# christhetree/mod_extraction

Hardware: NVIDIA B200
Metric: audio_seconds_rendered_per_second (higher is better)
Workload: dtype f32

## Files before the change

### mod_extraction_b200/csrc/phaser.cu

```cuda
#include "common.cuh"

namespace modfx {
namespace {

constexpr int kStagesAP = 6;
constexpr int kUpd = 4;
constexpr int kChunk = 128;
constexpr int kCtl = kChunk / kUpd;
constexpr int kState = 7;
constexpr int kMapFloats = 8 * kState;
constexpr int kSFloats = 8;

struct PhaserArgs {
    const float* x;
    float* y;
    int N;
    float sr;
    const float *rate, *depth, *centre, *feedback, *mix;
    int block;
    const int32_t* index;
    int n_items;
    int n_ctl;
    int n_chunks;
};

__device__ __forceinline__ int example_of(const PhaserArgs& a, int item) { return a.index ? a.index[item] : item; }

__device__ __forceinline__ float cascade_step(float in, float (&w)[kStagesAP], float c) {
    float v = in;
#pragma unroll
    for (int k = 0; k < kStagesAP; ++k) {
        const float y = fmaf(c, v, w[k]);
        w[k] = fmaf(-c, y, v);
        v = y;
    }
    return v;
}

__device__ __forceinline__ void cascade_retune(float (&w)[kStagesAP], float c_old, float c_new) {
    const float r = __fdividef(1.0f - c_new, 1.0f - c_old);
#pragma unroll
    for (int k = 0; k < kStagesAP; ++k) w[k] *= r;
}

__device__ __forceinline__ float2 cascade_step2(float2 in, float2 (&w)[kStagesAP], float c) {
    const float2 c2 = make_float2(c, c), nc2 = make_float2(-c, -c);
    float2 v = in;
#pragma unroll
    for (int k = 0; k < kStagesAP; ++k) {
        const float2 y = __ffma2_rn(c2, v, w[k]);
        w[k] = __ffma2_rn(nc2, y, v);
        v = y;
    }
    return v;
}

__device__ __forceinline__ void cascade_retune2(float2 (&w)[kStagesAP], float c_old, float c_new) {
    const float r = __fdividef(1.0f - c_new, 1.0f - c_old);
    const float2 r2 = make_float2(r, r);
#pragma unroll
    for (int k = 0; k < kStagesAP; ++k) w[k] = __fmul2_rn(w[k], r2);
}

constexpr int kSegChunks = 32;
constexpr int kSeg = kSegChunks * kChunk;
constexpr int kSub = 64;
constexpr int kSubs = kSeg / kSub;
constexpr int kSubCtl = kSub / kUpd;
constexpr int kSegCtl = kSeg / kUpd;
constexpr int kFusedThreads = 256;
constexpr int kRec = 8;

struct FusedArgs {
    PhaserArgs a;
    const int32_t* start;
    int n_out;
    float* dry_out;
    int x_compact;
    const int64_t* x_offset;
    int n_seg;
    int* ticket;
    int* flags;
    float* rec;
    float2* ph;
    float* phc;
};

__device__ __forceinline__ float phase_advance(float p, float inc, float two_pi) {
    const float next = p + inc;
    const float wrapped = next - two_pi;
    return (next >= two_pi) ? wrapped : next;
}

__global__ void __launch_bounds__(128) phaser_phase_kernel(const FusedArgs f, int n_blocks) {
    const PhaserArgs& a = f.a;
    const int pair = blockIdx.x * blockDim.x + threadIdx.x;
    if (pair >= a.n_items * n_blocks) return;
    const int item = pair / n_blocks, blk = pair - item * n_blocks;
    const int b = example_of(a, item);
    const int need = f.start ? min(a.N, f.start[b] + f.n_out) : a.N;
    if ((int64_t)blk * a.block >= need) return;
    const float two_pi = MODFX_TWO_PI_F;
    const float sr_down = (float)((double)a.sr / (double)kUpd);
    const float inc = a.rate[b] * (two_pi / sr_down);
    float p = 0.0f;
    for (int i = 0; i < blk; ++i) {
        const int n_down = ((i + 1) * a.block + kUpd - 1) / kUpd - (i * a.block + kUpd - 1) / kUpd;
        float next = __fadd_rn(p, __fmul_rn(inc, (float)n_down));
        while (next >= two_pi) next -= two_pi;
        p = next;
    }
    const int s0 = blk * a.block, s1 = min(s0 + a.block, a.N);
    if (f.phc) {
        float* out = f.phc + (int64_t)item * a.n_ctl;
        for (int j = (s0 + kUpd - 1) / kUpd; j < (s1 + kUpd - 1) / kUpd; ++j) {
            out[j] = p;
            float next = p + inc;
            while (next >= two_pi) next -= two_pi;
            p = next;
        }
        return;
    }
    const int c0 = s0 / kChunk, c1 = (s1 + kChunk - 1) / kChunk;
    float2* out = f.ph + (int64_t)item * a.n_chunks;
    float prev = 0.0f;
    const bool small = inc < two_pi;
    for (int c = c0; c < c1; ++c) {
        out[c].x = p;
        if (c > c0 || blk == 0) out[c].y = prev;
        if (small) {
#pragma unroll 8
            for (int j = 0; j < kCtl; ++j) {
                prev = p;
                p = phase_advance(p, inc, two_pi);
            }
        } else {
            for (int j = 0; j < kCtl; ++j) {
                prev = p;
                float next = p + inc;
                while (next >= two_pi) next -= two_pi;
                p = next;
            }
        }
    }
    if (s1 - s0 == a.block && c1 < a.n_chunks) out[c1].y = prev;
}

__device__ __forceinline__ float phaser_coef(float phase, float vol, float ctr, float log_span, float log_min, float w0) {
    float lfo = sinf(phase - MODFX_PI_F) * vol + ctr;
    lfo = fminf(fmaxf(lfo, 0.0f), 1.0f);
    const float fc = exp10f(lfo * log_span + log_min);
    const float g = tanf(w0 * fc);
    return 2.0f * (g / (1.0f + g)) - 1.0f;
}

__global__ void __launch_bounds__(kFusedThreads) phaser_fused_kernel(const FusedArgs f) {
    extern __shared__ __align__(16) float sm[];
    float(*xs)[kSub + 1] = reinterpret_cast<float(*)[kSub + 1]>(sm);
    float(*cs)[kSubCtl + 1] = reinterpret_cast<float(*)[kSubCtl + 1]>(sm + kSubs * (kSub + 1));
    float(*Ms)[kMapFloats + 1] = reinterpret_cast<float(*)[kMapFloats + 1]>(sm + kSubs * (kSub + 1) + kSubs * (kSubCtl + 1));
    float(*Ss)[kSFloats] = reinterpret_cast<float(*)[kSFloats]>(sm + kSubs * (kSub + 1) + kSubs * (kSubCtl + 1) + kSubs * (kMapFloats + 1));
    float* phs = reinterpret_cast<float*>(Ms);
    __shared__ int tile_s;
    __shared__ float entry[kRec];
    const PhaserArgs& a = f.a;
    const int tid = threadIdx.x, lane = tid & 31, warp = tid >> 5;
    if (tid == 0) tile_s = atomicAdd(f.ticket, 1);
    __syncthreads();
    const int tile = tile_s;
    const int seg = tile / a.n_items, item = tile - seg * a.n_items;
    const int b = example_of(a, item);
    const int start = f.start ? f.start[b] : 0;
    const int need = min(a.N, start + f.n_out);
    const int n_base = seg * kSeg;
    if (n_base >= need) return;
    const float* xr = f.x_offset ? a.x + f.x_offset[item] : a.x + (int64_t)(f.x_compact ? item : b) * a.N;
    const int row_len = f.x_offset ? need : a.N;

    const bool vec = ((reinterpret_cast<uintptr_t>(xr) & 15) == 0) && (n_base + kSeg <= row_len);
    if (vec) {
#pragma unroll
        for (int k = 0; k < kSeg / 4 / kFusedThreads; ++k) {
            const int i4 = tid + k * kFusedThreads;
            const float4 v = __ldg(reinterpret_cast<const float4*>(xr + n_base) + i4);
            float* d = &xs[i4 >> 4][(i4 & 15) << 2];
            d[0] = v.x; d[1] = v.y; d[2] = v.z; d[3] = v.w;
        }
    } else {
        for (int i = tid; i < kSeg; i += kFusedThreads) {
            const int n = n_base + i;
            xs[i / kSub][i % kSub] = (n < row_len) ? __ldg(xr + n) : 0.0f;
        }
    }
    const float two_pi = MODFX_TWO_PI_F;
    if (f.phc) {
        const float* pr = f.phc + (int64_t)item * a.n_ctl;
        for (int i = tid; i <= kSegCtl; i += kFusedThreads) {
            const int j = seg * kSegCtl - 1 + i;
            phs[i] = (j >= 0 && j < a.n_ctl) ? pr[j] : 0.0f;
        }
    } else if (tid < kSegChunks) {
        const int chunk = seg * kSegChunks + tid;
        const float sr_down = (float)((double)a.sr / (double)kUpd);
        const float inc = a.rate[b] * (two_pi / sr_down);
        float2 pp = (chunk < a.n_chunks) ? f.ph[(int64_t)item * a.n_chunks + chunk] : make_float2(0.0f, 0.0f);
        if (tid == 0) phs[0] = pp.y;
        float p = pp.x;
        if (inc < two_pi) {
#pragma unroll 8
            for (int q = 0; q < kCtl; ++q) {
                phs[1 + tid * kCtl + q] = p;
                p = phase_advance(p, inc, two_pi);
            }
        } else {
            for (int q = 0; q < kCtl; ++q) {
                phs[1 + tid * kCtl + q] = p;
                float next = p + inc;
                while (next >= two_pi) next -= two_pi;
                p = next;
            }
        }
    }
    __syncthreads();
    {
        const float f_lo = 20.0f;
        const double f_hi_d = (0.49 * (double)a.sr < 20000.0) ? 0.49 * (double)a.sr : 20000.0;
        const float log_min = log10f(f_lo), log_span = log10f((float)f_hi_d) - log_min;
        const float w0 = MODFX_PI_F / a.sr;
        const float vol = a.depth[b] * 0.5f;
        const float ctr = (log10f(a.centre[b]) - log_min) / log_span;
        float cv[(kSegCtl + 1 + kFusedThreads - 1) / kFusedThreads];
#pragma unroll
        for (int k = 0; k < (kSegCtl + 1 + kFusedThreads - 1) / kFusedThreads; ++k) {
            const int j = tid + k * kFusedThreads;
            cv[k] = (j <= kSegCtl) ? phaser_coef(phs[j], vol, ctr, log_span, log_min, w0) : 0.0f;
        }
        __syncthreads();
#pragma unroll
        for (int k = 0; k < (kSegCtl + 1 + kFusedThreads - 1) / kFusedThreads; ++k) {
            const int j = tid + k * kFusedThreads;
            if (j <= kSegCtl) {
                if (j >= 1) cs[(j - 1) / kSubCtl][1 + (j - 1) % kSubCtl] = cv[k];
                if (j % kSubCtl == 0 && j < kSegCtl) cs[j / kSubCtl][0] = cv[k];
            }
        }
    }
    __syncthreads();
    const float fbk = a.feedback[b];
    {
        const int pair = warp >> 1, sc = ((warp & 1) << 5) | lane;
        float2 s[kStagesAP];
#pragma unroll
        for (int k = 0; k < kStagesAP; ++k) s[k] = make_float2((2 * pair == k) ? 1.0f : 0.0f, (2 * pair + 1 == k) ? 1.0f : 0.0f);
        float2 out_prev = make_float2(0.0f, 0.0f);
        const float2 nfb = make_float2(-fbk, -fbk);
        float c_cur = cs[sc][0];
        int g0 = 0;
        if (pair == 3) {
            const float c0 = cs[sc][1];
            out_prev = cascade_step2(make_float2(-1.0f, xs[sc][0]), s, c0);
#pragma unroll
            for (int q = 1; q < kUpd; ++q)
                out_prev = cascade_step2(__ffma2_rn(nfb, out_prev, make_float2(0.0f, xs[sc][q])), s, c0);
            c_cur = c0;
            g0 = 1;
        }
#pragma unroll 2
        for (int g = g0; g < kSubCtl; ++g) {
            const float c = cs[sc][1 + g];
            cascade_retune2(s, c_cur, c);
            c_cur = c;
#pragma unroll
            for (int q = 0; q < kUpd; ++q) {
                const float2 u = (pair == 3) ? __ffma2_rn(nfb, out_prev, make_float2(0.0f, xs[sc][g * kUpd + q]))
                                             : __fmul2_rn(nfb, out_prev);
                out_prev = cascade_step2(u, s, c);
            }
        }
        float* m = &Ms[sc][2 * pair * kState];
#pragma unroll
        for (int k = 0; k < kStagesAP; ++k) {
            m[k] = s[k].x;
            m[kState + k] = s[k].y;
        }
        m[6] = out_prev.x * fbk;
        m[kState + 6] = out_prev.y * fbk;
    }
    __syncthreads();
    float(*GM)[kMapFloats + 1] = reinterpret_cast<float(*)[kMapFloats + 1]>(Ss + kSubs);
    float(*GS)[kSFloats] = reinterpret_cast<float(*)[kSFloats]>(reinterpret_cast<float*>(GM) + 8 * (kMapFloats + 1));
    {
        const int r = lane & 7, i0 = lane >> 3, i1 = i0 + 4;
        float* g = GM[warp];
        {
            const float* m = Ms[warp * 8];
            g[r * kState + i0] = m[r * kState + i0];
            if (i1 < kState) g[r * kState + i1] = m[r * kState + i1];
        }
        __syncwarp();
#pragma unroll 1
        for (int k = 1; k < 8; ++k) {
            const float* m = Ms[warp * 8 + k];
            float a0 = (r == 7) ? m[7 * kState + i0] : 0.0f;
            float a1 = (r == 7 && i1 < kState) ? m[7 * kState + i1] : 0.0f;
#pragma unroll
            for (int j = 0; j < kState; ++j) {
                const float cj = g[r * kState + j];
                a0 = fmaf(m[j * kState + i0], cj, a0);
                if (i1 < kState) a1 = fmaf(m[j * kState + i1], cj, a1);
            }
            __syncwarp();
            g[r * kState + i0] = a0;
            if (i1 < kState) g[r * kState + i1] = a1;
            __syncwarp();
        }
    }
    __syncthreads();
    if (warp == 0) {
        float* rec = f.rec + ((int64_t)item * f.n_seg + seg) * kRec;
        if (seg > 0) {
            const int* flag = f.flags + (int64_t)item * f.n_seg + seg - 1;
            if (lane == 0) {
                while (atomicAdd(const_cast<int*>(flag), 0) == 0) __nanosleep(64);
                __threadfence();
            }
            __syncwarp();
            if (lane < kRec) entry[lane] = __ldcg(rec - kRec + lane);
        } else if (lane < kRec) {
            entry[lane] = 0.0f;
        }
        __syncwarp();
        const int i = lane & 7, ii = (i < kState) ? i : 0;
        float sv = (i < kState) ? entry[i] : 0.0f;
        if (lane < 8) {
#pragma unroll 1
            for (int gq = 0; gq < 8; ++gq) {
                GS[gq][i] = sv;
                const float* m = GM[gq];
                float acc = m[7 * kState + ii];
#pragma unroll
                for (int r = 0; r < kState; ++r) acc = fmaf(m[r * kState + ii], __shfl_sync(0xffu, sv, r, 8), acc);
                sv = (i < kState) ? acc : 0.0f;
            }
            if (i < kState) rec[i] = sv;
            else rec[7] = cs[kSubs - 1][kSubCtl];
            __threadfence();
        }
        __syncwarp();
        if (lane == 0) atomicExch(f.flags + (int64_t)item * f.n_seg + seg, 1);
    }
    if (f.dry_out) {
        float* dr = f.dry_out + (int64_t)b * f.n_out;
        for (int i = tid; i < kSeg; i += kFusedThreads) {
            const int idx = n_base + i - start;
            if (idx >= 0 && idx < f.n_out && n_base + i < row_len) dr[idx] = xs[i / kSub][i % kSub];
        }
    }
    __syncthreads();
    if (lane < 8) {
        const int i = lane, ii = (i < kState) ? i : 0;
        float sv = (i < kState) ? GS[warp][i] : 0.0f;
#pragma unroll 1
        for (int k = 0; k < 8; ++k) {
            const int sc = warp * 8 + k;
            Ss[sc][i] = sv;
            const float* m = Ms[sc];
            float acc = m[7 * kState + ii];
#pragma unroll
            for (int r = 0; r < kState; ++r) acc = fmaf(m[r * kState + ii], __shfl_sync(0xffu, sv, r, 8), acc);
            sv = (i < kState) ? acc : 0.0f;
        }
    }
    __syncthreads();
    if (tid < kSubs) {
        const int sc = tid;
        float s[kStagesAP];
#pragma unroll
        for (int k = 0; k < kStagesAP; ++k) s[k] = Ss[sc][k];
        float last = Ss[sc][6];
        const float wet = a.mix[b], dry = 1.0f - a.mix[b];
        float c_cur = cs[sc][0];
#pragma unroll 2
        for (int g = 0; g < kSubCtl; ++g) {
            const float c = cs[sc][1 + g];
            cascade_retune(s, c_cur, c);
            c_cur = c;
#pragma unroll
            for (int q = 0; q < kUpd; ++q) {
                const float in = xs[sc][g * kUpd + q];
                const float out = cascade_step(in - last, s, c);
                last = out * fbk;
                xs[sc][g * kUpd + q] = fminf(fmaxf(fmaf(wet, out, dry * in), -1.0f), 1.0f);
            }
        }
    }
    __syncthreads();
    float* yr = a.y + (int64_t)b * f.n_out;
    if (vec && start == 0 && n_base + kSeg <= f.n_out && ((reinterpret_cast<uintptr_t>(yr) & 15) == 0)) {
#pragma unroll
        for (int k = 0; k < kSeg / 4 / kFusedThreads; ++k) {
            const int i4 = tid + k * kFusedThreads;
            const float* d = &xs[i4 >> 4][(i4 & 15) << 2];
            reinterpret_cast<float4*>(yr + n_base)[i4] = make_float4(d[0], d[1], d[2], d[3]);
        }
    } else {
        for (int i = tid; i < kSeg; i += kFusedThreads) {
            const int n = n_base + i;
            const int idx = n - start;
            if (idx >= 0 && idx < f.n_out && n < a.N) yr[idx] = xs[i / kSub][i % kSub];
        }
    }
}

int64_t align_up(int64_t v, int64_t a) { return (v + a - 1) / a * a; }

}
}

using namespace modfx;

extern "C" int64_t modfx_phaser_workspace_bytes(int32_t B, int64_t N) {
    if (B <= 0 || N <= 0) return 0;
    const int64_t n_ctl = (N + kUpd - 1) / kUpd, n_chunks = (N + kChunk - 1) / kChunk;
    const int64_t n_seg = (N + kSeg - 1) / kSeg;
    const int64_t phase_bytes = (n_ctl * 4 > n_chunks * 8) ? n_ctl * 4 : n_chunks * 8;
    return 256 + align_up((int64_t)B * n_seg * 4, 256) + align_up((int64_t)B * n_seg * kRec * 4, 256) +
           align_up((int64_t)B * phase_bytes, 256) + 256;
}

namespace {

int phaser_launch(const float* x, int x_compact, const int64_t* x_offset, float* y, float* dry_out, int32_t B, int64_t N, int64_t n_out, const int32_t* start,
                  float sr, const float* rate_hz, const float* depth, const float* centre_hz, const float* feedback,
                  const float* mix, int32_t block, const int32_t* example_index, int32_t n_items, void* workspace,
                  void* stream) {
    MODFX_REQUIRE(x && y && rate_hz && depth && centre_hz && feedback && mix, "NULL pointer");
    MODFX_REQUIRE(B >= 0 && N >= 1 && N < (1ll << 30), "bad shape B=%d N=%lld", B, (long long)N);
    MODFX_REQUIRE(n_out >= 1 && n_out <= N, "bad output window n_out=%lld (row length %lld)", (long long)n_out, (long long)N);
    MODFX_REQUIRE(sr > 0.0f, "sample rate must be positive");
    if (block <= 0) block = 8192;
    PhaserArgs a{};
    a.x = x; a.y = y; a.N = (int)N; a.sr = sr;
    a.rate = rate_hz; a.depth = depth; a.centre = centre_hz; a.feedback = feedback; a.mix = mix;
    a.block = block;
    a.index = example_index;
    a.n_items = example_index ? n_items : B;
    if (a.n_items == 0) return MODFX_OK;
    MODFX_REQUIRE(a.n_items > 0 && workspace, "workspace is NULL or n_items=%d", a.n_items);
    a.n_ctl = (int)((N + kUpd - 1) / kUpd);
    a.n_chunks = (int)((N + kChunk - 1) / kChunk);
    cudaStream_t s = as_stream(stream);
    char* w = static_cast<char*>(workspace);
    const int n_blocks = (int)((N + block - 1) / block);

    FusedArgs f{};
    f.a = a;
    f.start = start; f.n_out = (int)n_out; f.dry_out = dry_out; f.x_compact = x_compact; f.x_offset = x_offset;
    f.n_seg = (int)((N + kSeg - 1) / kSeg);
    f.ticket = reinterpret_cast<int*>(w);                                     w += 256;
    f.flags = reinterpret_cast<int*>(w);
    const int64_t flag_bytes = align_up((int64_t)a.n_items * f.n_seg * 4, 256);  w += flag_bytes;
    f.rec = reinterpret_cast<float*>(w);                                      w += align_up((int64_t)a.n_items * f.n_seg * kRec * 4, 256);
    if (block % kChunk == 0) f.ph = reinterpret_cast<float2*>(w);
    else f.phc = reinterpret_cast<float*>(w);
    MODFX_CUDA_OK(cudaMemsetAsync(workspace, 0, (size_t)(256 + flag_bytes), s));
    const int pairs = a.n_items * n_blocks;
    phaser_phase_kernel<<<(pairs + 127) / 128, 128, 0, s>>>(f, n_blocks);
    const size_t smem = sizeof(float) * (size_t)(kSubs * (kSub + 1) + kSubs * (kSubCtl + 1) + kSubs * (kMapFloats + 1) + kSubs * kSFloats +
                                                 8 * (kMapFloats + 1) + 8 * kSFloats);
    const int64_t tiles = (int64_t)a.n_items * f.n_seg;
    MODFX_REQUIRE(tiles < (1ll << 31), "too many segments in one call");
    phaser_fused_kernel<<<(unsigned)tiles, kFusedThreads, smem, s>>>(f);
    MODFX_CUDA_OK(cudaGetLastError());
    return MODFX_OK;
}

}

extern "C" int modfx_phaser_f32(const float* x, float* y, int32_t B, int64_t N, float sr, const float* rate_hz,
                                const float* depth, const float* centre_hz, const float* feedback,
                                const float* mix, int32_t block, const int32_t* example_index, int32_t n_items,
                                void* workspace, void* stream) {
    return phaser_launch(x, 0, nullptr, y, nullptr, B, N, N, nullptr, sr, rate_hz, depth, centre_hz, feedback, mix, block, example_index,
                         n_items, workspace, stream);
}

extern "C" int modfx_phaser_crop_f32(const float* x, int32_t x_compact, float* y, float* dry_out, int32_t B, int64_t N,
                                     int64_t n_out, const int32_t* start, float sr, const float* rate_hz, const float* depth,
                                     const float* centre_hz, const float* feedback, const float* mix, int32_t block,
                                     const int32_t* example_index, int32_t n_items, void* workspace, void* stream) {
    MODFX_REQUIRE(start, "start is NULL");
    MODFX_REQUIRE(!x_compact || example_index, "x_compact needs an example_index list");
    return phaser_launch(x, x_compact ? 1 : 0, nullptr, y, dry_out, B, N, n_out, start, sr, rate_hz, depth, centre_hz, feedback, mix, block, example_index,
                         n_items, workspace, stream);
}

extern "C" int modfx_phaser_crop_packed_f32(const float* x, const int64_t* x_offset, float* y, float* dry_out, int32_t B,
                                            int64_t N_max, int64_t n_out, const int32_t* start, float sr, const float* rate_hz,
                                            const float* depth, const float* centre_hz, const float* feedback, const float* mix,
                                            int32_t block, const int32_t* example_index, int32_t n_items, void* workspace,
                                            void* stream) {
    MODFX_REQUIRE(start && x_offset, "start or x_offset is NULL");
    MODFX_REQUIRE(example_index, "a packed x needs an example_index list (row i belongs to example example_index[i])");
    return phaser_launch(x, 1, x_offset, y, dry_out, B, N_max, n_out, start, sr, rate_hz, depth, centre_hz, feedback, mix, block,
                         example_index, n_items, workspace, stream);
}
```

Measured before the change: 1.214 million.

## Split final phaser replay into two pieces per sub-chunk and precompute retune ratios

Retune ratios are precomputed once into shared memory, so the per-step division in the transfer-map pass goes away. The map pass also records boundary states at the sub-chunk midpoint. These are combined with the entry state so that two warps replay the final wet pass in parallel per sub-chunk, each covering half the length. Segments that lie entirely before the start offset now return early, and the launch bound requests 5 blocks per SM. The cost is more register pressure from the boundary state arrays, extra shared-memory partial sums, and one more barrier.

New measurement: 1.245 million (median of 6 runs). 1.03x the previous value.

```diff
diff --git a/mod_extraction_b200/csrc/phaser.cu b/mod_extraction_b200/csrc/phaser.cu
--- a/mod_extraction_b200/csrc/phaser.cu
+++ b/mod_extraction_b200/csrc/phaser.cu
@@ -55,8 +55,7 @@
     return v;
 }
 
-__device__ __forceinline__ void cascade_retune2(float2 (&w)[kStagesAP], float c_old, float c_new) {
-    const float r = __fdividef(1.0f - c_new, 1.0f - c_old);
+__device__ __forceinline__ void cascade_rescale2(float2 (&w)[kStagesAP], float r) {
     const float2 r2 = make_float2(r, r);
 #pragma unroll
     for (int k = 0; k < kStagesAP; ++k) w[k] = __fmul2_rn(w[k], r2);
@@ -68,6 +67,9 @@
 constexpr int kSubs = kSeg / kSub;
 constexpr int kSubCtl = kSub / kUpd;
 constexpr int kSegCtl = kSeg / kUpd;
+constexpr int kPieces = 2;
+constexpr int kPieceLen = kSub / kPieces;
+constexpr int kPieceCtl = kSubCtl / kPieces;
 constexpr int kFusedThreads = 256;
 constexpr int kRec = 8;
 
@@ -154,7 +156,32 @@
     return 2.0f * (g / (1.0f + g)) - 1.0f;
 }
 
-__global__ void __launch_bounds__(kFusedThreads) phaser_fused_kernel(const FusedArgs f) {
+template <bool kAudio>
+__device__ __forceinline__ void map_runs(float2 (&s)[kStagesAP], float2& out_prev, int g0, const float* xrow,
+                                         const float* crow, const float* rcol, float fbk, float2 (&bd)[kPieces - 1][kState]) {
+    const float2 nfb = make_float2(-fbk, -fbk);
+#pragma unroll
+    for (int pc = 0; pc < kPieces; ++pc) {
+#pragma unroll 1
+        for (int g = (pc == 0) ? g0 : pc * kPieceCtl; g < (pc + 1) * kPieceCtl; ++g) {
+            const float c = crow[1 + g];
+            cascade_rescale2(s, rcol[g * kSubs]);
+#pragma unroll
+            for (int q = 0; q < kUpd; ++q) {
+                const float2 u = kAudio ? __ffma2_rn(nfb, out_prev, make_float2(0.0f, xrow[g * kUpd + q]))
+                                        : __fmul2_rn(nfb, out_prev);
+                out_prev = cascade_step2(u, s, c);
+            }
+        }
+        if (pc + 1 < kPieces) {
+#pragma unroll
+            for (int k = 0; k < kStagesAP; ++k) bd[pc][k] = s[k];
+            bd[pc][6] = __fmul2_rn(out_prev, make_float2(fbk, fbk));
+        }
+    }
+}
+
+__global__ void __launch_bounds__(kFusedThreads, 5) phaser_fused_kernel(const FusedArgs f) {
     extern __shared__ __align__(16) float sm[];
     float(*xs)[kSub + 1] = reinterpret_cast<float(*)[kSub + 1]>(sm);
     float(*cs)[kSubCtl + 1] = reinterpret_cast<float(*)[kSubCtl + 1]>(sm + kSubs * (kSub + 1));
@@ -246,36 +273,31 @@
         }
     }
     __syncthreads();
+    float* rs = &Ss[0][0];
+    static_assert(kSubCtl * kSubs <= kSubs * kSFloats + 8 * (kMapFloats + 1 + kSFloats), "rs does not fit over Ss, GM and GS");
+    for (int i = tid; i < kSubCtl * kSubs; i += kFusedThreads) {
+        const int g = i / kSubs, r = i % kSubs;
+        rs[i] = __fdividef(1.0f - cs[r][1 + g], 1.0f - cs[r][g]);
+    }
+    __syncthreads();
     const float fbk = a.feedback[b];
+    const int pair = warp >> 1, sc = ((warp & 1) << 5) | lane;
+    float2 bd[kPieces - 1][kState];
     {
-        const int pair = warp >> 1, sc = ((warp & 1) << 5) | lane;
         float2 s[kStagesAP];
 #pragma unroll
         for (int k = 0; k < kStagesAP; ++k) s[k] = make_float2((2 * pair == k) ? 1.0f : 0.0f, (2 * pair + 1 == k) ? 1.0f : 0.0f);
         float2 out_prev = make_float2(0.0f, 0.0f);
-        const float2 nfb = make_float2(-fbk, -fbk);
-        float c_cur = cs[sc][0];
-        int g0 = 0;
         if (pair == 3) {
+            const float2 nfb = make_float2(-fbk, -fbk);
             const float c0 = cs[sc][1];
             out_prev = cascade_step2(make_float2(-1.0f, xs[sc][0]), s, c0);
 #pragma unroll
             for (int q = 1; q < kUpd; ++q)
                 out_prev = cascade_step2(__ffma2_rn(nfb, out_prev, make_float2(0.0f, xs[sc][q])), s, c0);
-            c_cur = c0;
-            g0 = 1;
-        }
-#pragma unroll 2
-        for (int g = g0; g < kSubCtl; ++g) {
-            const float c = cs[sc][1 + g];
-            cascade_retune2(s, c_cur, c);
-            c_cur = c;
-#pragma unroll
-            for (int q = 0; q < kUpd; ++q) {
-                const float2 u = (pair == 3) ? __ffma2_rn(nfb, out_prev, make_float2(0.0f, xs[sc][g * kUpd + q]))
-                                             : __fmul2_rn(nfb, out_prev);
-                out_prev = cascade_step2(u, s, c);
-            }
+            map_runs<true>(s, out_prev, 1, xs[sc], cs[sc], rs + sc, fbk, bd);
+        } else {
+            map_runs<false>(s, out_prev, 0, xs[sc], cs[sc], rs + sc, fbk, bd);
         }
         float* m = &Ms[sc][2 * pair * kState];
 #pragma unroll
@@ -349,6 +371,7 @@
         __syncwarp();
         if (lane == 0) atomicExch(f.flags + (int64_t)item * f.n_seg + seg, 1);
     }
+    if (n_base + kSeg <= start) return;
     if (f.dry_out) {
         float* dr = f.dry_out + (int64_t)b * f.n_out;
         for (int i = tid; i < kSeg; i += kFusedThreads) {
@@ -372,16 +395,42 @@
         }
     }
     __syncthreads();
-    if (tid < kSubs) {
-        const int sc = tid;
+    float st[kState];
+    {
+        float* part = &Ms[0][0];
+        const float sa = Ss[sc][2 * pair], sb = (pair == 3) ? 1.0f : Ss[sc][2 * pair + 1];
+        if (pair == 0) {
+#pragma unroll
+            for (int i = 0; i < kState; ++i) st[i] = Ss[sc][i];
+        }
+        static_assert((kPieces - 1) * 3 * kState * kSubs <= kSubs * (kMapFloats + 1), "piece entry terms do not fit over Ms");
+#pragma unroll
+        for (int p = 1; p < kPieces; ++p) {
+#pragma unroll
+            for (int i = 0; i < kState; ++i) {
+                const float v = fmaf(bd[p - 1][i].x, sa, bd[p - 1][i].y * sb);
+                if (pair == p) st[i] = v;
+                else part[(((p - 1) * 3 + pair - (pair > p)) * kState + i) * kSubs + sc] = v;
+            }
+        }
+        __syncthreads();
+        if (pair > 0 && pair < kPieces) {
+#pragma unroll
+            for (int j = 0; j < 3; ++j) {
+#pragma unroll
+                for (int i = 0; i < kState; ++i) st[i] += part[(((pair - 1) * 3 + j) * kState + i) * kSubs + sc];
+            }
+        }
+    }
+    if (pair < kPieces && n_base + sc * kSub + (pair + 1) * kPieceLen > start) {
         float s[kStagesAP];
 #pragma unroll
-        for (int k = 0; k < kStagesAP; ++k) s[k] = Ss[sc][k];
-        float last = Ss[sc][6];
+        for (int k = 0; k < kStagesAP; ++k) s[k] = st[k];
+        float last = st[6];
         const float wet = a.mix[b], dry = 1.0f - a.mix[b];
-        float c_cur = cs[sc][0];
+        float c_cur = cs[sc][pair * kPieceCtl];
 #pragma unroll 2
-        for (int g = 0; g < kSubCtl; ++g) {
+        for (int g = pair * kPieceCtl; g < (pair + 1) * kPieceCtl; ++g) {
             const float c = cs[sc][1 + g];
             cascade_retune(s, c_cur, c);
             c_cur = c;
```

## Shrink fused phaser smem, keep warp map composition in registers, raise occupancy

Applied to the files above, without the earlier changes.

Removes the GM/GS shared scratch buffers. The per-warp affine-map composition now keeps its running product in registers and reads it through shuffles, and the composed maps and entry states are written back into the existing Ms/Ss slots. Launch bounds request 6 CTAs per SM, and the carveout is set to maximum shared memory so more tiles can be resident at once. Coefficient constants are computed once per block by one thread and shared, and the dry and wet window stores are vectorised over only the valid range, with an early exit for segments that lie entirely before the crop start. The risks are register pressure from the occupancy target and an extra cudaFuncSetAttribute call on every launch.

After: 1.215 million before, 1.255 million after (median of 6 runs). 3.2% higher.

```diff
diff --git a/mod_extraction_b200/csrc/phaser.cu b/mod_extraction_b200/csrc/phaser.cu
--- a/mod_extraction_b200/csrc/phaser.cu
+++ b/mod_extraction_b200/csrc/phaser.cu
@@ -69,7 +69,10 @@
 constexpr int kSubCtl = kSub / kUpd;
 constexpr int kSegCtl = kSeg / kUpd;
 constexpr int kFusedThreads = 256;
+constexpr int kFusedCtasPerSM = 6;
 constexpr int kRec = 8;
+constexpr int kFusedSmemFloats = kSubs * (kSub + 1) + kSubs * (kSubCtl + 1) + kSubs * (kMapFloats + 1) + kSubs * kSFloats;
+static_assert(kFusedCtasPerSM * (kFusedSmemFloats * 4 + 128 + 1024) <= 228 * 1024, "phaser_fused_kernel: 6 CTAs per SM");
 
 struct FusedArgs {
     PhaserArgs a;
@@ -154,7 +157,21 @@
     return 2.0f * (g / (1.0f + g)) - 1.0f;
 }
 
-__global__ void __launch_bounds__(kFusedThreads) phaser_fused_kernel(const FusedArgs f) {
+__device__ __forceinline__ void store_window(float* row, const float (*xs)[kSub + 1], int n_base, int start, int lo, int hi,
+                                             int tid) {
+    const auto at = [&](int n) { const unsigned i = n - n_base; return xs[i / kSub][i % kSub]; };
+    if ((reinterpret_cast<uintptr_t>(row) & 15) != 0) {
+        for (int n = lo + tid; n < hi; n += kFusedThreads) row[n - start] = at(n);
+        return;
+    }
+    const int v0 = min(lo + ((start - lo) & 3), hi), v1 = max(hi - ((hi - start) & 3), v0);
+    for (int n = v0 + 4 * tid; n < v1; n += 4 * kFusedThreads)
+        *reinterpret_cast<float4*>(row + (n - start)) = make_float4(at(n), at(n + 1), at(n + 2), at(n + 3));
+    if (tid < v0 - lo) row[lo + tid - start] = at(lo + tid);
+    if (tid < hi - v1) row[v1 + tid - start] = at(v1 + tid);
+}
+
+__global__ void __launch_bounds__(kFusedThreads, kFusedCtasPerSM) phaser_fused_kernel(const FusedArgs f) {
     extern __shared__ __align__(16) float sm[];
     float(*xs)[kSub + 1] = reinterpret_cast<float(*)[kSub + 1]>(sm);
     float(*cs)[kSubCtl + 1] = reinterpret_cast<float(*)[kSubCtl + 1]>(sm + kSubs * (kSub + 1));
@@ -163,6 +180,7 @@
     float* phs = reinterpret_cast<float*>(Ms);
     __shared__ int tile_s;
     __shared__ float entry[kRec];
+    __shared__ float coef_k[5];
     const PhaserArgs& a = f.a;
     const int tid = threadIdx.x, lane = tid & 31, warp = tid >> 5;
     if (tid == 0) tile_s = atomicAdd(f.ticket, 1);
@@ -191,6 +209,16 @@
             const int n = n_base + i;
             xs[i / kSub][i % kSub] = (n < row_len) ? __ldg(xr + n) : 0.0f;
         }
+    }
+    if (tid == kFusedThreads - 1) {
+        const float f_lo = 20.0f;
+        const double f_hi_d = (0.49 * (double)a.sr < 20000.0) ? 0.49 * (double)a.sr : 20000.0;
+        const float log_min = log10f(f_lo), log_span = log10f((float)f_hi_d) - log_min;
+        coef_k[0] = log_min;
+        coef_k[1] = log_span;
+        coef_k[2] = MODFX_PI_F / a.sr;
+        coef_k[3] = a.depth[b] * 0.5f;
+        coef_k[4] = (log10f(a.centre[b]) - log_min) / log_span;
     }
     const float two_pi = MODFX_TWO_PI_F;
     if (f.phc) {
@@ -223,12 +251,7 @@
     }
     __syncthreads();
     {
-        const float f_lo = 20.0f;
-        const double f_hi_d = (0.49 * (double)a.sr < 20000.0) ? 0.49 * (double)a.sr : 20000.0;
-        const float log_min = log10f(f_lo), log_span = log10f((float)f_hi_d) - log_min;
-        const float w0 = MODFX_PI_F / a.sr;
-        const float vol = a.depth[b] * 0.5f;
-        const float ctr = (log10f(a.centre[b]) - log_min) / log_span;
+        const float log_min = coef_k[0], log_span = coef_k[1], w0 = coef_k[2], vol = coef_k[3], ctr = coef_k[4];
         float cv[(kSegCtl + 1 + kFusedThreads - 1) / kFusedThreads];
 #pragma unroll
         for (int k = 0; k < (kSegCtl + 1 + kFusedThreads - 1) / kFusedThreads; ++k) {
@@ -287,17 +310,14 @@
         m[kState + 6] = out_prev.y * fbk;
     }
     __syncthreads();
-    float(*GM)[kMapFloats + 1] = reinterpret_cast<float(*)[kMapFloats + 1]>(Ss + kSubs);
-    float(*GS)[kSFloats] = reinterpret_cast<float(*)[kSFloats]>(reinterpret_cast<float*>(GM) + 8 * (kMapFloats + 1));
     {
         const int r = lane & 7, i0 = lane >> 3, i1 = i0 + 4;
-        float* g = GM[warp];
+        float g0, g1;
         {
             const float* m = Ms[warp * 8];
-            g[r * kState + i0] = m[r * kState + i0];
-            if (i1 < kState) g[r * kState + i1] = m[r * kState + i1];
-        }
-        __syncwarp();
+            g0 = m[r * kState + i0];
+            g1 = (i1 < kState) ? m[r * kState + i1] : 0.0f;
+        }
 #pragma unroll 1
         for (int k = 1; k < 8; ++k) {
             const float* m = Ms[warp * 8 + k];
@@ -305,15 +325,17 @@
             float a1 = (r == 7 && i1 < kState) ? m[7 * kState + i1] : 0.0f;
 #pragma unroll
             for (int j = 0; j < kState; ++j) {
-                const float cj = g[r * kState + j];
+                const float cj = __shfl_sync(0xffffffffu, (j < 4) ? g0 : g1, ((j & 3) << 3) | r);
                 a0 = fmaf(m[j * kState + i0], cj, a0);
                 if (i1 < kState) a1 = fmaf(m[j * kState + i1], cj, a1);
             }
-            __syncwarp();
-            g[r * kState + i0] = a0;
-            if (i1 < kState) g[r * kState + i1] = a1;
-            __syncwarp();
-        }
+            g0 = a0;
+            g1 = a1;
+        }
+        __syncwarp();
+        float* g = Ms[warp * 8 + 7];
+        g[r * kState + i0] = g0;
+        if (i1 < kState) g[r * kState + i1] = g1;
     }
     __syncthreads();
     if (warp == 0) {
@@ -335,8 +357,8 @@
         if (lane < 8) {
 #pragma unroll 1
             for (int gq = 0; gq < 8; ++gq) {
-                GS[gq][i] = sv;
-                const float* m = GM[gq];
+                Ss[gq * 8][i] = sv;
+                const float* m = Ms[gq * 8 + 7];
                 float acc = m[7 * kState + ii];
 #pragma unroll
                 for (int r = 0; r < kState; ++r) acc = fmaf(m[r * kState + ii], __shfl_sync(0xffu, sv, r, 8), acc);
@@ -349,26 +371,22 @@
         __syncwarp();
         if (lane == 0) atomicExch(f.flags + (int64_t)item * f.n_seg + seg, 1);
     }
-    if (f.dry_out) {
-        float* dr = f.dry_out + (int64_t)b * f.n_out;
-        for (int i = tid; i < kSeg; i += kFusedThreads) {
-            const int idx = n_base + i - start;
-            if (idx >= 0 && idx < f.n_out && n_base + i < row_len) dr[idx] = xs[i / kSub][i % kSub];
-        }
-    }
+    if (n_base + kSeg <= start) return;
+    const int lo = max(n_base, start), hi = min(n_base + kSeg, need);
+    if (f.dry_out) store_window(f.dry_out + (int64_t)b * f.n_out, xs, n_base, start, lo, hi, tid);
     __syncthreads();
     if (lane < 8) {
         const int i = lane, ii = (i < kState) ? i : 0;
-        float sv = (i < kState) ? GS[warp][i] : 0.0f;
+        float sv = (i < kState) ? Ss[warp * 8][i] : 0.0f;
 #pragma unroll 1
-        for (int k = 0; k < 8; ++k) {
+        for (int k = 0; k < 7; ++k) {
             const int sc = warp * 8 + k;
-            Ss[sc][i] = sv;
             const float* m = Ms[sc];
             float acc = m[7 * kState + ii];
 #pragma unroll
             for (int r = 0; r < kState; ++r) acc = fmaf(m[r * kState + ii], __shfl_sync(0xffu, sv, r, 8), acc);
             sv = (i < kState) ? acc : 0.0f;
+            Ss[sc + 1][i] = sv;
         }
     }
     __syncthreads();
@@ -396,7 +414,7 @@
     }
     __syncthreads();
     float* yr = a.y + (int64_t)b * f.n_out;
-    if (vec && start == 0 && n_base + kSeg <= f.n_out && ((reinterpret_cast<uintptr_t>(yr) & 15) == 0)) {
+    if (start == 0 && n_base + kSeg <= f.n_out && ((reinterpret_cast<uintptr_t>(yr) & 15) == 0)) {
 #pragma unroll
         for (int k = 0; k < kSeg / 4 / kFusedThreads; ++k) {
             const int i4 = tid + k * kFusedThreads;
@@ -404,11 +422,7 @@
             reinterpret_cast<float4*>(yr + n_base)[i4] = make_float4(d[0], d[1], d[2], d[3]);
         }
     } else {
-        for (int i = tid; i < kSeg; i += kFusedThreads) {
-            const int n = n_base + i;
-            const int idx = n - start;
-            if (idx >= 0 && idx < f.n_out && n < a.N) yr[idx] = xs[i / kSub][i % kSub];
-        }
+        store_window(yr, xs, n_base, start, lo, hi, tid);
     }
 }
 
@@ -466,11 +480,11 @@
     MODFX_CUDA_OK(cudaMemsetAsync(workspace, 0, (size_t)(256 + flag_bytes), s));
     const int pairs = a.n_items * n_blocks;
     phaser_phase_kernel<<<(pairs + 127) / 128, 128, 0, s>>>(f, n_blocks);
-    const size_t smem = sizeof(float) * (size_t)(kSubs * (kSub + 1) + kSubs * (kSubCtl + 1) + kSubs * (kMapFloats + 1) + kSubs * kSFloats +
-                                                 8 * (kMapFloats + 1) + 8 * kSFloats);
     const int64_t tiles = (int64_t)a.n_items * f.n_seg;
     MODFX_REQUIRE(tiles < (1ll << 31), "too many segments in one call");
-    phaser_fused_kernel<<<(unsigned)tiles, kFusedThreads, smem, s>>>(f);
+    MODFX_CUDA_OK(cudaFuncSetAttribute(phaser_fused_kernel, cudaFuncAttributePreferredSharedMemoryCarveout,
+                                       cudaSharedmemCarveoutMaxShared));
+    phaser_fused_kernel<<<(unsigned)tiles, kFusedThreads, sizeof(float) * kFusedSmemFloats, s>>>(f);
     MODFX_CUDA_OK(cudaGetLastError());
     return MODFX_OK;
 }
```
